# argmaxinc/WhisperKit

Measured on NVIDIA H100. Metric: RTFx (audio-sec/s) whisper-large-v3 greedy, higher is better.
Workload: dtype bf16

## Files before the change

### include/wkb200.h

```cpp
#ifndef WKB200_H
#define WKB200_H

#include <stdint.h>

#ifdef __cplusplus
extern "C" {
#endif

typedef int32_t wk_status;
enum {
    WK_OK = 0,
    WK_ERR_INVALID_ARGUMENT = -1,
    WK_ERR_MODELS_UNAVAILABLE = -2,
    WK_ERR_AUDIO_PROCESSING_FAILED = -3,
    WK_ERR_PREPARE_DECODER_INPUTS = -4,
    WK_ERR_DECODING_LOGITS_FAILED = -5,
    WK_ERR_DECODING_FAILED = -6,
    WK_ERR_TRANSCRIPTION_FAILED = -7,
    WK_ERR_CUDA = -8,
    WK_ERR_LOAD_AUDIO_FAILED = -9
};

typedef struct wk_model wk_model;
typedef struct wk_session wk_session;
// ... 254 lines not shown
                                               int64_t seek, float last_speech_timestamp, float constrained_median, float max_duration,
                                               int32_t special_token_begin, const wk_tokenizer_hooks* hooks, wk_words** out);
wk_status wk_add_word_timestamps(wk_segment* segs, int32_t n_segs, const int32_t* tokens, const float* token_logprobs,
                                 const void* alignment, int32_t dtype, int32_t rows, int32_t cols, int64_t ld,
                                 const wk_tokenizer_hooks* hooks, int64_t seek, float last_speech_timestamp, int32_t special_token_begin,
                                 const char* prepended, const char* appended, wk_words** out);

typedef struct wk_tokenizer wk_tokenizer;
wk_status wk_tokenizer_load(const char* path, wk_tokenizer** out);
wk_status wk_tokenizer_create(const char* const* tokens, const int32_t* ids, const uint8_t* flags, int32_t n, int32_t clean_up_tokenization_spaces,
                              wk_tokenizer** out);
void wk_tokenizer_free(wk_tokenizer* t);
int32_t wk_tokenizer_vocab_size(const wk_tokenizer* t);
int32_t wk_tokenizer_token_to_id(const wk_tokenizer* t, const char* token);
int32_t wk_tokenizer_decode(const wk_tokenizer* t, const int32_t* tokens, int32_t n, int32_t skip_special_tokens, char* text, int32_t cap);
int32_t wk_tokenizer_encode(const wk_tokenizer* t, const char* text_utf8, int32_t* ids, int32_t cap);
wk_status wk_tokenizer_set_merges(wk_tokenizer* t, const char* const* left, const char* const* right, int32_t n);
wk_status wk_tokenizer_special_tokens(const wk_tokenizer* t, wk_special_tokens* out);
int32_t wk_tokenizer_split_to_word_tokens(const wk_tokenizer* t, const int32_t* tokens, int32_t n, char* text, int32_t text_cap, int32_t* counts,
                                          int32_t counts_cap);
wk_status wk_tokenizer_hooks_init(wk_tokenizer* t, wk_tokenizer_hooks* hooks);

int32_t wk_format_time(float seconds, int32_t always_include_hours, const char* decimal_marker, char* out, int32_t cap);
int32_t wk_write_srt(const float* starts, const float* ends, const char* const* texts, int32_t n, char* out, int32_t cap);
int32_t wk_write_vtt(const float* starts, const float* ends, const char* const* texts, int32_t n, char* out, int32_t cap);

int64_t wk_kernel_launch_count(int32_t reset);
wk_status wk_last_timings(wk_model* m, float* ms6);
void* wk_model_stream(wk_model* m);

wk_status wk_test_gemm(wk_model* m, const void* a, const void* w, const float* bias, void* out, int32_t M, int32_t N, int32_t K,
                       int32_t in_dtype, int32_t out_dtype, int32_t gelu);
wk_status wk_test_gemm_residual(wk_model* m, const void* a, const void* w, const float* bias, float* out, int32_t M, int32_t N, int32_t K, int32_t in_dtype);
wk_status wk_test_gemm_splitk(wk_model* m, const void* w, const void* x, float* out, int32_t N, int32_t rows_x, int32_t K, int32_t in_dtype, int32_t splits);
wk_status wk_test_attention(wk_model* m, const void* qkv, void* out, int32_t B, int32_t T, int32_t n_heads, int32_t dtype);
wk_status wk_test_cross_attention(wk_model* m, const float* q, const void* kcross, const void* vcross, void* out, int32_t B, int32_t H,
                                  int32_t T, int32_t dtype, const int32_t* done);
wk_status wk_test_cross_attention_shared(wk_model* m, const float* q, const void* kcross, const void* vcross, void* out, int32_t B, int32_t H,
                                         int32_t T, int32_t dtype, const int32_t* done, int32_t kv_div);
wk_status wk_test_cross_attention_fp8(wk_model* m, const float* q, const uint8_t* kcodes, const uint8_t* vcodes, const float* kscale,
                                      const float* vscale, void* out, int32_t B, int32_t H, int32_t T, int32_t dtype, const int32_t* done,
                                      int32_t kv_div, float* align_out);
wk_status wk_test_self_attention(wk_model* m, const float* qkv, void* kcache, void* vcache, const int32_t* pos, void* out, int32_t B,
                                 int32_t H, int32_t dtype, const int32_t* done);
wk_status wk_test_gemm_partial(wk_model* m, const void* w, const void* x, float* partial_out, int32_t N, int32_t rows_x, int32_t partial_cols,
                               int32_t K, int32_t dtype, int32_t splits);
wk_status wk_test_decoder_reduce(wk_model* m, int32_t kind, const float* partial, int32_t splits, int32_t Bp, const float* bias, const float* gamma,
                                 const float* beta, float* x, void* out16, int32_t B, int32_t n, int32_t dtype);
wk_status wk_test_self_attention_splitk(wk_model* m, const float* partial, int32_t splits, int32_t Bp, const float* bq, const float* bv, void* kcache,
                                        void* vcache, const int32_t* pos, const int32_t* done, const int32_t* anc, void* out, int32_t B, int32_t H,
                                        int32_t dtype);
wk_status wk_test_cross_attention_splitk(wk_model* m, const float* partial, int32_t splits, int32_t Bp, const float* bq, const void* kcross,
                                         const void* vcross, const float* kscale, const float* vscale, void* out, int32_t B, int32_t H, int32_t T,
                                         int32_t dtype, const int32_t* done, int32_t kv_div);

wk_status wk_bench_kernel(wk_model* m, wk_session* s, int32_t which, int32_t batch, int32_t iters, float* ms_out, double* work_out);

wk_status wk_debug_read(wk_model* m, wk_session* s, int32_t which, int64_t offset_elems, float* dst, int64_t n);

#ifdef __cplusplus
}
#endif
#endif
```

### whisperkit_b200/_lib.py

```python
from __future__ import annotations

import ctypes as C
import os

_PKG = os.path.dirname(os.path.abspath(__file__))
LIB_PATH = os.path.join(_PKG, "libwkb200.so")

WK_DTYPE_F32, WK_DTYPE_F16, WK_DTYPE_BF16, WK_DTYPE_I32 = 0, 1, 2, 3
WK_DTYPE_FP8_E4M3 = 4

STATUS_NAMES = {
    0: "ok", -1: "invalidArgument", -2: "modelsUnavailable", -3: "audioProcessingFailed",
    -4: "prepareDecoderInputsFailed", -5: "decodingLogitsFailed", -6: "decodingFailed",
    -7: "transcriptionFailed", -8: "cudaError", -9: "loadAudioFailed",
}
WK_ERR_INVALID_ARGUMENT, WK_ERR_LOAD_AUDIO_FAILED = -1, -9
WK_AUDIO_U8, WK_AUDIO_S16, WK_AUDIO_S24, WK_AUDIO_S32, WK_AUDIO_F32 = 0, 1, 2, 3, 4
WK_CHANNELS_SUM, WK_CHANNELS_SPECIFIC = 0, 1


class WhisperError(RuntimeError):

    def __init__(self, status: int, message: str):
        super().__init__(f"{STATUS_NAMES.get(status, status)}: {message}")
# ... 177 lines not shown
    ("wk_dtw", I32, [P, I32, I32, I32, I64, PI32, PI32, I32, PI32]),
    ("wk_find_alignment", I32, [C.POINTER(wk_word), I32, P, I32, I32, I32, I64, PF32, I32, C.POINTER(P)]),
    ("wk_merge_punctuations", I32, [C.POINTER(wk_word), I32, C.c_char_p, C.c_char_p, C.POINTER(P)]),
    ("wk_word_duration_constraints", I32, [C.POINTER(wk_word), I32, PF32, PF32]),
    ("wk_truncate_long_words", I32, [C.POINTER(wk_word), I32, F32, C.POINTER(P)]),
    ("wk_update_segments_with_word_timings", I32, [C.POINTER(wk_segment), I32, PI32, C.POINTER(wk_word), I32, I64, F32, F32, F32, I32,
                                                   C.POINTER(wk_tokenizer_hooks), C.POINTER(P)]),
    ("wk_add_word_timestamps", I32, [C.POINTER(wk_segment), I32, PI32, PF32, P, I32, I32, I32, I64, C.POINTER(wk_tokenizer_hooks), I64, F32, I32,
                                     C.c_char_p, C.c_char_p, C.POINTER(P)]),
    ("wk_detect_variant", I32, [I32, I32, C.POINTER(C.c_char_p), C.POINTER(C.c_char_p), PI32]),
    ("wk_tokenizer_load", I32, [C.c_char_p, C.POINTER(P)]),
    ("wk_tokenizer_create", I32, [C.POINTER(C.c_char_p), PI32, C.POINTER(C.c_uint8), I32, I32, C.POINTER(P)]),
    ("wk_tokenizer_free", None, [P]),
    ("wk_tokenizer_vocab_size", I32, [P]),
    ("wk_tokenizer_token_to_id", I32, [P, C.c_char_p]),
    ("wk_tokenizer_decode", I32, [P, PI32, I32, I32, C.POINTER(C.c_char), I32]),
    ("wk_tokenizer_encode", I32, [P, C.c_char_p, PI32, I32]),
    ("wk_tokenizer_set_merges", I32, [P, C.POINTER(C.c_char_p), C.POINTER(C.c_char_p), I32]),
    ("wk_tokenizer_special_tokens", I32, [P, C.POINTER(wk_special_tokens)]),
    ("wk_tokenizer_split_to_word_tokens", I32, [P, PI32, I32, C.POINTER(C.c_char), I32, PI32, I32]),
    ("wk_tokenizer_hooks_init", I32, [P, C.POINTER(wk_tokenizer_hooks)]),
    ("wk_format_time", I32, [F32, I32, C.c_char_p, C.POINTER(C.c_char), I32]),
    ("wk_write_srt", I32, [PF32, PF32, C.POINTER(C.c_char_p), I32, C.POINTER(C.c_char), I32]),
    ("wk_write_vtt", I32, [PF32, PF32, C.POINTER(C.c_char_p), I32, C.POINTER(C.c_char), I32]),
    ("wk_kernel_launch_count", I64, [I32]),
    ("wk_last_timings", I32, [P, PF32]),
    ("wk_model_stream", P, [P]),
    ("wk_test_gemm", I32, [P, P, P, P, P, I32, I32, I32, I32, I32, I32]),
    ("wk_test_cross_attention", I32, [P, P, P, P, P, I32, I32, I32, I32, P]),
    ("wk_test_cross_attention_shared", I32, [P, P, P, P, P, I32, I32, I32, I32, P, I32]),
    ("wk_test_cross_attention_fp8", I32, [P, P, P, P, P, P, P, I32, I32, I32, I32, P, I32, P]),
    ("wk_test_self_attention", I32, [P, P, P, P, P, P, I32, I32, I32, P]),
    ("wk_test_gemm_residual", I32, [P, P, P, P, P, I32, I32, I32, I32]),
    ("wk_test_gemm_splitk", I32, [P, P, P, P, I32, I32, I32, I32, I32]),
    ("wk_test_attention", I32, [P, P, P, I32, I32, I32, I32]),
    ("wk_test_gemm_partial", I32, [P, P, P, P, I32, I32, I32, I32, I32, I32]),
    ("wk_test_decoder_reduce", I32, [P, I32, P, I32, I32, P, P, P, P, P, I32, I32, I32]),
    ("wk_test_self_attention_splitk", I32, [P, P, I32, I32, P, P, P, P, P, P, P, P, I32, I32, I32]),
    ("wk_test_cross_attention_splitk", I32, [P, P, I32, I32, P, P, P, P, P, P, I32, I32, I32, I32, P, I32]),
    ("wk_debug_read", I32, [P, P, I32, I64, P, I64]),
    ("wk_bench_kernel", I32, [P, P, I32, I32, I32, PF32, C.POINTER(C.c_double)]),
]

_lib = None


def load() -> C.CDLL:
    global _lib
    if _lib is not None:
        return _lib
    if not os.path.exists(LIB_PATH):
        raise ImportError(
            f"{LIB_PATH} not built: run `python -m whisperkit_b200.build` (needs nvcc). "
            "whisperkit_b200 has no CPU or PyTorch fallback.")
    lib = C.CDLL(LIB_PATH)
    for name, restype, argtypes in SYMBOLS:
        fn = getattr(lib, name)
        fn.restype = restype
        fn.argtypes = argtypes
    _lib = lib
    return lib


def check(status: int) -> None:
    if status != 0:
        raise WhisperError(status, load().wk_last_error().decode("utf-8", "replace"))
# ... 1 lines not shown
```

### whisperkit_b200/csrc/common.cuh

```cuda
#pragma once
#include <cuda.h>
#include <cuda_bf16.h>
#include <cuda_fp16.h>
#include <cuda_fp8.h>
#include <cuda_runtime.h>
#include <stdint.h>
#include <stdio.h>
#include <string.h>

namespace wk {

template <typename T> struct T16;
template <> struct T16<__nv_bfloat16> {
    __device__ __forceinline__ static float to_f(__nv_bfloat16 v) { return __bfloat162float(v); }
    __device__ __forceinline__ static __nv_bfloat16 from_f(float v) { return __float2bfloat16_rn(v); }
    __device__ __forceinline__ static uint32_t pack2(float a, float b) {
        __nv_bfloat162 t = __floats2bfloat162_rn(a, b);
        return *reinterpret_cast<uint32_t*>(&t);
    }
    __device__ __forceinline__ static float2 unpack2(uint32_t u) {
        __nv_bfloat162 t = *reinterpret_cast<__nv_bfloat162*>(&u);
        return __bfloat1622float2(t);
    }
};
// ... 148 lines not shown
}
__device__ __forceinline__ void tma_load_2d_elect(void* smem_dst, const void* tmap, uint64_t* bar, int c0, int c1) {
    asm volatile(
        "{\n\t.reg .pred q;\n\t"
        "elect.sync _|q, 0xffffffff;\n\t"
        "@q cp.async.bulk.tensor.2d.shared::cluster.global.tile.mbarrier::complete_tx::bytes [%0], [%1, {%3, %4}], [%2];\n\t}"
        ::"r"(smem_u32(smem_dst)), "l"(tmap), "r"(smem_u32(bar)), "r"(c0), "r"(c1)
        : "memory");
}
__device__ __forceinline__ void tma_load_3d_elect(void* smem_dst, const void* tmap, uint64_t* bar, int c0, int c1, int c2) {
    asm volatile(
        "{\n\t.reg .pred q;\n\t"
        "elect.sync _|q, 0xffffffff;\n\t"
        "@q cp.async.bulk.tensor.3d.shared::cluster.global.tile.mbarrier::complete_tx::bytes [%0], [%1, {%3, %4, %5}], [%2];\n\t}"
        ::"r"(smem_u32(smem_dst)), "l"(tmap), "r"(smem_u32(bar)), "r"(c0), "r"(c1), "r"(c2)
        : "memory");
}
__device__ __forceinline__ void mbar_expect_tx_elect(uint64_t* bar, uint32_t bytes) {
    asm volatile(
        "{\n\t.reg .pred q;\n\t"
        "elect.sync _|q, 0xffffffff;\n\t"
        "@q mbarrier.arrive.expect_tx.shared::cta.b64 _, [%0], %1;\n\t}" ::"r"(smem_u32(bar)), "r"(bytes)
        : "memory");
}
__device__ __forceinline__ void tma_store_3d(const void* tmap, const void* smem_src, int c0, int c1, int c2) {
    asm volatile("cp.async.bulk.tensor.3d.global.shared::cta.bulk_group [%0, {%2, %3, %4}], [%1];"
                 ::"l"(tmap), "r"(smem_u32(smem_src)), "r"(c0), "r"(c1), "r"(c2)
                 : "memory");
}
__device__ __forceinline__ void bulk_commit() { asm volatile("cp.async.bulk.commit_group;" ::: "memory"); }
__device__ __forceinline__ void bulk_wait_read_all() { asm volatile("cp.async.bulk.wait_group.read 0;" ::: "memory"); }
__device__ __forceinline__ void bulk_wait_all() { asm volatile("cp.async.bulk.wait_group 0;" ::: "memory"); }
__device__ __forceinline__ void warpgroup_bar(int id) { asm volatile("bar.sync %0, 128;" ::"r"(id) : "memory"); }
__device__ __forceinline__ void stmatrix_x4(uint32_t smem_addr, uint32_t r0, uint32_t r1, uint32_t r2, uint32_t r3) {
    asm volatile("stmatrix.sync.aligned.m8n8.x4.shared.b16 [%0], {%1, %2, %3, %4};" ::"r"(smem_addr), "r"(r0), "r"(r1), "r"(r2), "r"(r3)
                 : "memory");
}
__device__ __forceinline__ void bulk_load_1d(void* smem_dst, const void* gsrc, uint32_t bytes, uint64_t* bar) {
    asm volatile(
        "cp.async.bulk.shared::cluster.global.mbarrier::complete_tx::bytes [%0], [%1], %2, [%3];" ::"r"(
            smem_u32(smem_dst)),
        "l"(gsrc), "r"(bytes), "r"(smem_u32(bar))
        : "memory");
}

__device__ __forceinline__ void pdl_launch_dependents() { asm volatile("griddepcontrol.launch_dependents;" ::: "memory"); }
__device__ __forceinline__ void pdl_wait() { asm volatile("griddepcontrol.wait;" ::: "memory"); }

__device__ __forceinline__ void cp_async16(void* smem_dst, const void* gsrc, bool pred) {
    uint32_t sz = pred ? 16u : 0u;
    asm volatile("cp.async.cg.shared.global [%0], [%1], 16, %2;" ::"r"(smem_u32(smem_dst)), "l"(gsrc), "r"(sz)
                 : "memory");
}
__device__ __forceinline__ void cp_async_commit() { asm volatile("cp.async.commit_group;" ::: "memory"); }
template <int N> __device__ __forceinline__ void cp_async_wait() {
    asm volatile("cp.async.wait_group %0;" ::"n"(N) : "memory");
}

bool pdl_enabled();
int pdl_mode();
void pdl_disable();
template <typename... KArgs, typename... Args>
inline cudaError_t launch_k(void (*kernel)(KArgs...), dim3 grid, dim3 block, size_t smem, cudaStream_t stream, int pdl,
                            Args&&... args) {
    cudaLaunchConfig_t cfg;
    memset(&cfg, 0, sizeof(cfg));
// ... 23 lines not shown
```

### whisperkit_b200/csrc/engine.cu

```cuda
#include <math.h>
#include <stdarg.h>
#include <stdio.h>
#include <stdlib.h>
#include <string.h>
#include <dirent.h>

#include <algorithm>
#include <atomic>
#include <map>
#include <string>
#include <vector>

#include "common.cuh"
#include "engine.h"

namespace wk {

static thread_local char g_err[1024] = "";
void set_error(const char* fmt, ...) {
    va_list ap;
    va_start(ap, fmt);
    vsnprintf(g_err, sizeof(g_err), fmt, ap);
    va_end(ap);
}
// ... 884 lines not shown

int64_t wk_kernel_launch_count(int32_t reset) {
    const long long v = wk::launch_counter_load();
    if (reset) wk::launch_counter_sub(v);
    return v;
}

wk_status wk_last_timings(wk_model* m, float* ms6) {
    if (!m || !ms6) return WK_ERR_INVALID_ARGUMENT;
    memcpy(ms6, m->timings, sizeof(m->timings));
    return WK_OK;
}

wk_status wk_test_gemm(wk_model* m, const void* a, const void* w, const float* bias, void* out, int32_t M, int32_t N, int32_t K,
                       int32_t in_dtype, int32_t out_dtype, int32_t gelu) {
    if (!m) return WK_ERR_INVALID_ARGUMENT;
    WK_CUDA_CHECK(cudaSetDevice(m->device));
    std::lock_guard<std::mutex> lock(m->api_mu);
    const int mode = out_dtype == WK_DTYPE_F32 ? GEMM_OUT_F32 : GEMM_OUT_T16;
    WK_CHECK(gemm_wgmma(plain_gemm(a, M, K, w, N, in_dtype, mode, out, N, bias, gelu), m->num_sms, m->stream));
    WK_CUDA_CHECK(cudaStreamSynchronize(m->stream));
    return WK_OK;
}

wk_status wk_test_gemm_residual(wk_model* m, const void* a, const void* w, const float* bias, float* out, int32_t M, int32_t N, int32_t K, int32_t in_dtype) {
    if (!m || !a || !w || !out) return WK_ERR_INVALID_ARGUMENT;
    WK_CUDA_CHECK(cudaSetDevice(m->device));
    std::lock_guard<std::mutex> lock(m->api_mu);
    WK_CHECK(gemm_wgmma(plain_gemm(a, M, K, w, N, in_dtype, GEMM_OUT_F32_ADD, out, N, bias, 0), m->num_sms, m->stream));
    WK_CUDA_CHECK(cudaStreamSynchronize(m->stream));
    return WK_OK;
}

__global__ void reduce_partials_kernel(const float* __restrict__ partial, int splits, int Bp, int N, int rows, float* __restrict__ out) {
    const long long idx = (long long)blockIdx.x * blockDim.x + threadIdx.x;
    if (idx >= (long long)rows * N) return;
    const int b = (int)(idx / N), i = (int)(idx % N);
    float a = 0.f;
    for (int s = 0; s < splits; ++s) a += partial[((long long)s * Bp + b) * N + i];
    out[idx] = a;
}

wk_status wk_test_gemm_splitk(wk_model* m, const void* w, const void* x, float* out, int32_t N, int32_t rows_x, int32_t K, int32_t in_dtype, int32_t splits) {
    if (!m) return WK_ERR_INVALID_ARGUMENT;
    WK_CUDA_CHECK(cudaSetDevice(m->device));
    std::lock_guard<std::mutex> lock(m->api_mu);
    if (rows_x % 16 != 0 || rows_x > 256) { set_error("wk_test_gemm_splitk: rows_x must be a multiple of 16 <= 256"); return WK_ERR_INVALID_ARGUMENT; }
    const int tiles = (N + 127) / 128;
    const int sp = splits > 0 ? splits : choose_splits(tiles, K / 64, m->num_sms);
    float* partial = nullptr;
    WK_CUDA_CHECK(cudaMalloc(&partial, (size_t)sp * rows_x * N * 4));
    GemmDesc g;
    memset(&g, 0, sizeof(g));
    g.a = w; g.a_rows = N; g.a_cols = K; g.a_ld = K; g.a_batches = 1;
    g.b = x; g.b_rows = rows_x; g.b_ld = K; g.in_dtype = in_dtype;
    g.m_rows_per_batch = N; g.n = rows_x; g.k = K; g.taps = 1; g.bn = rows_x; g.splits = sp;
    g.mode = GEMM_OUT_PARTIAL_T; g.out = partial; g.ld_out = N; g.out_rows_per_batch = N; g.partial_cols = rows_x;
    wk_status r = gemm_wgmma(g, m->num_sms, m->stream);
    if (r == WK_OK) {
        const long long n = (long long)rows_x * N;
        reduce_partials_kernel<<<(unsigned)((n + 255) / 256), 256, 0, m->stream>>>(partial, sp, rows_x, N, rows_x, out);
        cudaError_t e = cudaStreamSynchronize(m->stream);
        if (e != cudaSuccess) { set_error("wk_test_gemm_splitk: %s", cudaGetErrorString(e)); r = WK_ERR_CUDA; }
    }
    cudaFree(partial);
    return r;
// ... 145 lines not shown
```

### whisperkit_b200/csrc/gemm_wgmma.cu

```cuda
#include <stdarg.h>
#include <stdio.h>
#include <stdlib.h>

#include <algorithm>

#include "common.cuh"
#include "kernels.h"
#include "wgmma.cuh"

namespace wk {

static constexpr int kBlockM = 128;
static constexpr int kBlockK = 64;
static constexpr int kStageA = kBlockM * kBlockK * 2;
static constexpr int kGemmThreads = 384;
static constexpr int kMaxStages = 10;
static constexpr int kSmemMax = 227 * 1024;

struct GemmKParams {
    int tiles_per_batch, n_batches, tiles_n, splits, work;
    int kb_per_tap, kb_per_split, taps;
    int tap_row_shift[3];
    int tap_col_off[3];
    int a_is_3d;
    int m_rows_per_batch, n, bn;
    int stage_b_bytes, stages, store_bytes;
    int mode, gelu;
    void* out;
    long long ld_out, out_rows_per_batch, partial_cols;
    const float* bias;
    const float* pos;
    long long ld_pos;
    int heads_T, heads_B, heads_H, heads_dmodel;
    float* out_scale;
    int a_static;
};

enum GemmEpi { kEpiPartialT = 0, kEpiFp8Heads = 1, kEpiStore16 = 2, kEpiStore32 = 3 };
static int gemm_epi(int mode) {
    switch (mode) {
        case GEMM_OUT_PARTIAL_T: return kEpiPartialT;
        case GEMM_OUT_FP8_HEADS: return kEpiFp8Heads;
        case GEMM_OUT_T16: case GEMM_OUT_T16_HEADS: return kEpiStore16;
        default: return kEpiStore32;
    }
}

static constexpr int kStoreBox = 64 * 128;
static constexpr int kStoreBytes = 2  * 2  * kStoreBox;

__device__ __forceinline__ uint32_t swz128(int row, int chunk) { return (uint32_t)(row * 128 + ((chunk ^ (row & 7)) << 4)); }

__device__ __forceinline__ void store_box_begin(int wg_tid, int cw) {
    fence_proxy_async();
    if (wg_tid == 0) bulk_wait_read_all();
    warpgroup_bar(1 + cw);
}

template <typename T, int BN>
__device__ __forceinline__ void gemm_epilogue_store16(const GemmKParams& p, const CUtensorMap* tmO, const float (&acc)[BN / 2],
                                                      uint8_t* stage, int& sbuf, int wg_tid, int cw, int batch, int row0, int col_base) {
    const int lane = wg_tid & 31;
    const int q = lane & 3;
    const int mrow = 16 * (wg_tid >> 5) + 8 * ((lane >> 3) & 1) + (lane & 7);
    const int mj = lane >> 4;
    const bool heads = p.mode == GEMM_OUT_T16_HEADS;
    int hb = 0, ht0 = 0;
    bool straddle = false;
// ... 287 lines not shown
            }
            prev = stage;
            if (++stage == p.stages) { stage = 0; phase ^= 1; }
        }
        wgmma_wait<0>();
        __syncwarp();
        if (lane == 0) mbar_arrive(&empty_bar[prev]);

        if constexpr (EPI == kEpiFp8Heads) {
            gemm_epilogue_fp8_heads<BN>(p, batch, tile_row0, r_lo, c_lo, col_base, acc);
        } else if constexpr (EPI == kEpiStore16) {
            if (wg_rows) gemm_epilogue_store16<T, BN>(p, &tmO, acc, my_stage, sbuf, wg_tid, cw, batch, wg_row0, col_base);
        } else if constexpr (EPI == kEpiStore32) {
            if (wg_rows) gemm_epilogue_store32<BN>(p, &tmO, acc, my_stage, my_res_bar, sbuf, rphase, wg_tid, cw, batch, wg_row0, col_base);
        } else {
            float* o = reinterpret_cast<float*>(p.out);
#pragma unroll
            for (int half = 0; half < 2; ++half) {
                const int row_in_batch = tile_row0 + r_lo + 8 * half;
                if (row_in_batch >= p.m_rows_per_batch) continue;
                const long long grow = (long long)batch * p.out_rows_per_batch + row_in_batch;
#pragma unroll
                for (int j = 0; j < BN / 8; ++j) {
                    const int col = col_base + 8 * j + c_lo;
                    if (col < p.partial_cols) o[((long long)split * p.partial_cols + col) * p.ld_out + grow] = acc[4 * j + 2 * half];
                    if (col + 1 < p.partial_cols) o[((long long)split * p.partial_cols + col + 1) * p.ld_out + grow] = acc[4 * j + 2 * half + 1];
                }
            }
        }
    }
    if (kStore && wg_tid == 0) bulk_wait_all();
}

typedef CUresult (*PFN_encodeTiled)(CUtensorMap*, CUtensorMapDataType, cuuint32_t, void*, const cuuint64_t*, const cuuint64_t*,
                                    const cuuint32_t*, const cuuint32_t*, CUtensorMapInterleave, CUtensorMapSwizzle,
                                    CUtensorMapL2promotion, CUtensorMapFloatOOBfill);

static PFN_encodeTiled get_encode_fn() {
    static PFN_encodeTiled fn = nullptr;
    if (!fn) {
        void* p = nullptr;
        cudaDriverEntryPointQueryResult q;
        if (cudaGetDriverEntryPoint("cuTensorMapEncodeTiled", &p, cudaEnableDefault, &q) == cudaSuccess &&
            q == cudaDriverEntryPointSuccess)
            fn = reinterpret_cast<PFN_encodeTiled>(p);
    }
    return fn;
}

static wk_status make_tmap(CUtensorMap* tm, const void* base, int dtype, int ndim, const uint64_t* dims,
                           const uint64_t* strides_bytes, const uint32_t* box) {
    PFN_encodeTiled enc = get_encode_fn();
    if (!enc) {
        set_error("cuTensorMapEncodeTiled entry point unavailable (no CUDA driver?)");
        return WK_ERR_CUDA;
    }
    cuuint64_t gdim[3];
    cuuint64_t gstr[2];
    cuuint32_t bx[3];
    cuuint32_t es[3] = {1, 1, 1};
    for (int i = 0; i < ndim; ++i) { gdim[i] = dims[i]; bx[i] = box[i]; }
    for (int i = 0; i < ndim - 1; ++i) gstr[i] = strides_bytes[i];
    const CUtensorMapDataType ty = dtype == WK_DTYPE_F32 ? CU_TENSOR_MAP_DATA_TYPE_FLOAT32
                                   : dtype == WK_DTYPE_F16 ? CU_TENSOR_MAP_DATA_TYPE_FLOAT16 : CU_TENSOR_MAP_DATA_TYPE_BFLOAT16;
    CUresult r = enc(tm, ty,
                     (cuuint32_t)ndim, const_cast<void*>(base), gdim, gstr, bx, es, CU_TENSOR_MAP_INTERLEAVE_NONE,
// ... 30 lines not shown
        attr_set = true;
    }
    return launch_k(gemm_wgmma_kernel<T, BN, EPI>, dim3(grid), dim3(kGemmThreads), smem, stream, pdl, tmA, tmB, tmO, p);
}

template <typename T, int EPI>
static cudaError_t launch_gemm_store(const CUtensorMap& tmA, const CUtensorMap& tmB, const CUtensorMap& tmO, const GemmKParams& p, int grid,
                                     size_t smem, int pdl, cudaStream_t stream) {
    switch (p.bn) {
        case 64: return launch_gemm<T, 64, EPI>(tmA, tmB, tmO, p, grid, smem, pdl, stream);
        case 128: return launch_gemm<T, 128, EPI>(tmA, tmB, tmO, p, grid, smem, pdl, stream);
        default: return launch_gemm<T, 256, EPI>(tmA, tmB, tmO, p, grid, smem, pdl, stream);
    }
}

template <typename T>
static cudaError_t launch_gemm_n(const CUtensorMap& tmA, const CUtensorMap& tmB, const CUtensorMap& tmO, const GemmKParams& p, int grid,
                                 size_t smem, int pdl, cudaStream_t stream) {
    switch (gemm_epi(p.mode)) {
        case kEpiFp8Heads: return launch_gemm<T, 256, kEpiFp8Heads>(tmA, tmB, tmO, p, grid, smem, pdl, stream);
        case kEpiStore16: return launch_gemm_store<T, kEpiStore16>(tmA, tmB, tmO, p, grid, smem, pdl, stream);
        case kEpiStore32: return launch_gemm_store<T, kEpiStore32>(tmA, tmB, tmO, p, grid, smem, pdl, stream);
        default: break;
    }
    switch (p.bn) {
        case 16: return launch_gemm<T, 16, kEpiPartialT>(tmA, tmB, tmO, p, grid, smem, pdl, stream);
        case 32: return launch_gemm<T, 32, kEpiPartialT>(tmA, tmB, tmO, p, grid, smem, pdl, stream);
        case 64: return launch_gemm<T, 64, kEpiPartialT>(tmA, tmB, tmO, p, grid, smem, pdl, stream);
        case 128: return launch_gemm<T, 128, kEpiPartialT>(tmA, tmB, tmO, p, grid, smem, pdl, stream);
        default: return launch_gemm<T, 256, kEpiPartialT>(tmA, tmB, tmO, p, grid, smem, pdl, stream);
    }
}

wk_status gemm_wgmma(const GemmDesc& d, int num_sms, cudaStream_t stream) {
    if (d.k % kBlockK != 0 || d.bn % 16 != 0 || d.bn < 16 || d.bn > 256 || d.taps < 1 || d.taps > 3) {
        set_error("gemm_wgmma: unsupported shape k=%d bn=%d taps=%d", d.k, d.bn, d.taps);
        return WK_ERR_INVALID_ARGUMENT;
    }
    if (d.mode != GEMM_OUT_PARTIAL_T && (d.n % 32 != 0 || d.splits != 1)) {
        set_error("gemm_wgmma: n=%d must be a multiple of 32 and splits 1 for mode %d", d.n, d.mode);
        return WK_ERR_INVALID_ARGUMENT;
    }
    GemmKParams p;
    memset(&p, 0, sizeof(p));
    p.kb_per_tap = d.k / kBlockK;
    const int total_kb = p.kb_per_tap * d.taps;
    p.splits = d.splits < 1 ? 1 : d.splits;
    if (total_kb % p.splits != 0) {
        set_error("gemm_wgmma: splits %d does not divide %d k-blocks", p.splits, total_kb);
        return WK_ERR_INVALID_ARGUMENT;
    }
    p.kb_per_split = total_kb / p.splits;
    p.taps = d.taps;
    for (int i = 0; i < 3; ++i) { p.tap_row_shift[i] = d.tap_row_shift[i]; p.tap_col_off[i] = d.tap_col_off[i]; }
    p.a_is_3d = d.a_3d ? 1 : 0;
    p.n_batches = d.a_3d ? d.a_batches : 1;
    p.m_rows_per_batch = d.m_rows_per_batch;
    p.tiles_per_batch = (d.m_rows_per_batch + kBlockM - 1) / kBlockM;
    p.n = d.n;
    p.bn = wgmma_tile_n(d.bn);
    const int epi = gemm_epi(d.mode);
    const bool tma_store = epi == kEpiStore16 || epi == kEpiStore32;
    if (tma_store && p.bn < 64) p.bn = 64;
    p.tiles_n = (d.n + p.bn - 1) / p.bn;
    p.work = p.tiles_per_batch * p.n_batches * p.tiles_n * p.splits;
    p.stage_b_bytes = p.bn * kBlockK * 2;
    if (p.stage_b_bytes % 1024 != 0) p.stage_b_bytes = (p.stage_b_bytes + 1023) / 1024 * 1024;
    const int stage_bytes = kStageA + p.stage_b_bytes;
    p.store_bytes = tma_store ? kStoreBytes : 0;
    const int smem_budget = kSmemMax - 1024  - 256  - p.store_bytes;
    int stages = smem_budget / stage_bytes;
    if (stages > kMaxStages) stages = kMaxStages;
    if (stages > total_kb / p.splits + 2) stages = total_kb / p.splits + 2;
    if (stages < 2) stages = 2;
    if (d.max_stages > 0 && stages > d.max_stages) stages = d.max_stages;
    p.stages = stages;
    p.a_static = d.a_static;
    p.mode = d.mode;
    p.gelu = d.gelu;
    p.out = d.out;
    p.ld_out = d.ld_out;
    p.out_rows_per_batch = d.out_rows_per_batch;
    p.partial_cols = d.partial_cols;
    p.bias = d.bias;
    p.pos = d.pos;
    p.ld_pos = d.ld_pos;
    p.heads_T = d.heads_T; p.heads_B = d.heads_B; p.heads_H = d.heads_H; p.heads_dmodel = d.heads_dmodel;
    p.out_scale = d.out_scale;
    if (d.mode == GEMM_OUT_FP8_HEADS && (p.bn != 256 || d.n % 64 != 0 || d.heads_dmodel % 64 != 0 || !d.out_scale)) {
        set_error("gemm_wgmma: the FP8 heads epilogue needs 256-column tiles and head-aligned columns (bn %d n %d d %d)", p.bn, d.n, d.heads_dmodel);
        return WK_ERR_INVALID_ARGUMENT;
    }
    if (d.mode == GEMM_OUT_T16_HEADS &&
        (p.n_batches != 1 || d.n % 64 != 0 || d.heads_dmodel % 64 != 0 || d.n % d.heads_dmodel != 0 || d.m_rows_per_batch % d.heads_T != 0)) {
        set_error("gemm_wgmma: the 16-bit heads epilogue needs head-aligned columns and whole windows (n %d d %d rows %d T %d)", d.n,
                  d.heads_dmodel, d.m_rows_per_batch, d.heads_T);
        return WK_ERR_INVALID_ARGUMENT;
    }

    CUtensorMap tmA, tmB, tmO;
    memset(&tmO, 0, sizeof(tmO));
    wk_status st;
    if (p.a_is_3d) {
        uint64_t dims[3] = {(uint64_t)d.a_cols, (uint64_t)d.a_rows, (uint64_t)d.a_batches};
        uint64_t str[2] = {(uint64_t)d.a_ld * 2, (uint64_t)d.a_batch_stride * 2};
        uint32_t box[3] = {kBlockK, kBlockM, 1};
        st = make_tmap(&tmA, d.a, d.in_dtype, 3, dims, str, box);
    } else {
        uint64_t dims[2] = {(uint64_t)d.a_cols, (uint64_t)d.a_rows};
        uint64_t str[1] = {(uint64_t)d.a_ld * 2};
        uint32_t box[2] = {kBlockK, kBlockM};
        st = make_tmap(&tmA, d.a, d.in_dtype, 2, dims, str, box);
    }
    if (st != WK_OK) return st;
    {
        uint64_t dims[2] = {(uint64_t)d.k * d.taps, (uint64_t)d.b_rows};
        uint64_t str[1] = {(uint64_t)d.b_ld * 2};
        uint32_t box[2] = {kBlockK, (uint32_t)p.bn};
        st = make_tmap(&tmB, d.b, d.in_dtype, 2, dims, str, box);
        if (st != WK_OK) return st;
    }
    if (d.mode == GEMM_OUT_T16_HEADS) {
        uint64_t dims[3] = {64, (uint64_t)d.heads_T, (uint64_t)(d.n / d.heads_dmodel) * d.heads_B * d.heads_H};
        uint64_t str[2] = {128, (uint64_t)d.heads_T * 128};
        uint32_t box[3] = {64, 64, 1};
        st = make_tmap(&tmO, d.out, d.in_dtype, 3, dims, str, box);
    } else if (tma_store) {
        const int out_dtype = epi == kEpiStore16 ? d.in_dtype : WK_DTYPE_F32;
        const uint64_t es = epi == kEpiStore16 ? 2 : 4;
        uint64_t dims[3] = {(uint64_t)d.n, (uint64_t)d.m_rows_per_batch, (uint64_t)p.n_batches};
        uint64_t str[2] = {(uint64_t)d.ld_out * es, (uint64_t)d.out_rows_per_batch * d.ld_out * es};
        uint32_t box[3] = {(uint32_t)(128 / es), 64, 1};
        st = make_tmap(&tmO, d.out, out_dtype, 3, dims, str, box);
    }
    if (st != WK_OK) return st;
    const size_t smem_bytes = (size_t)stages * stage_bytes + p.store_bytes + 1024 + 256;
    int grid = p.work < num_sms ? p.work : num_sms;
    if (grid < 1) return WK_OK;
    const int pdl = d.pdl != 0 ? 16 : 0;
    cudaError_t e = d.in_dtype == WK_DTYPE_F16 ? launch_gemm_n<__half>(tmA, tmB, tmO, p, grid, smem_bytes, pdl, stream)
                                               : launch_gemm_n<__nv_bfloat16>(tmA, tmB, tmO, p, grid, smem_bytes, pdl, stream);
    count_launch();
    if (e == cudaSuccess) e = cudaGetLastError();
    if (e != cudaSuccess) {
        set_error("gemm_wgmma launch: %s", cudaGetErrorString(e));
        return WK_ERR_CUDA;
    }
    return WK_OK;
}

}
```

### whisperkit_b200/csrc/kernels.h

```cpp
#pragma once
#include <cuda.h>
#include <cuda_runtime.h>
#include <stdint.h>

#include "../../include/wkb200.h"

namespace wk {

void set_error(const char* fmt, ...);
const char* last_error_cstr();
void count_launch(int n = 1);

enum GemmMode {
    GEMM_OUT_T16 = 0,
    GEMM_OUT_F32_ADD = 1,
    GEMM_OUT_F32_GELU_POS = 2,
    GEMM_OUT_PARTIAL_T = 3,
    GEMM_OUT_T16_HEADS = 4,
    GEMM_OUT_F32 = 5,
    GEMM_OUT_FP8_HEADS = 6,
};

struct GemmDesc {
    const void* a;
    int64_t a_rows;
    int64_t a_cols;
    int64_t a_ld;
    int64_t a_batch_stride;
    int a_batches;
    int a_3d;
    const void* b;
    int64_t b_rows;
    int64_t b_ld;
    int in_dtype;
    int m_rows_per_batch;
    int n;
    int k;
    int taps;
    int tap_row_shift[3];
    int tap_col_off[3];
    int bn;
    int splits;
    int mode;
    int gelu;
    void* out;
    int64_t ld_out;
    int64_t out_rows_per_batch;
    int64_t partial_cols;
    const float* bias;
    const float* pos;
    int64_t ld_pos;
    int heads_T, heads_B, heads_H, heads_dmodel;
    float* out_scale;
    int pdl;
    int max_stages;
    int a_static;
};

wk_status gemm_wgmma(const GemmDesc& d, int num_sms, cudaStream_t stream);
int wgmma_tile_n(int bn);

struct MelTables;
wk_status mel_tables_create(int n_mels, MelTables** out);
void mel_tables_free(MelTables* t);
wk_status mel_forward(const MelTables* t, const float* pcm, int64_t n_windows, int64_t stride, const int32_t* n_valid,
                      void* out_f16, int32_t* gmax_scratch, cudaStream_t stream);
constexpr int kMelRows = 3002;
constexpr int kMelCols = 128;

wk_status layernorm_f32_to_16(const float* x, const float* gamma, const float* beta, void* out, int64_t rows, int d, int dtype,
                              cudaStream_t stream);
wk_status layernorm_f32_to_f32(const float* x, const float* gamma, const float* beta, float* out, int64_t rows, int d,
                               cudaStream_t stream);
wk_status encoder_attention(const void* qkv, void* out, int B, int T, int n_heads, int dtype, cudaStream_t stream);
wk_status encoder_attention_wgmma(const void* qkv, void* out, int B, int T, int n_heads, int dtype, cudaStream_t stream);
wk_status transpose_to_host_layout(const void* src, float* dst, int64_t B, int64_t rows, int64_t cols, int64_t src_rows_alloc,
                                   int64_t src_row_off, int64_t src_ld, int dtype, cudaStream_t stream);
wk_status fill_random_16(void* dst, int64_t n, uint64_t seed, float std, float mean, int dtype, cudaStream_t stream);
wk_status fill_random_f32(float* dst, int64_t n, uint64_t seed, float std, float mean, cudaStream_t stream);
wk_status convert_to_16(const void* src, int src_dtype, void* dst, int dst_dtype, int64_t n, cudaStream_t stream);

struct RowParams {
    int32_t prompt_len;
    int32_t sample_begin_ts;
    int32_t sample_begin_blank;
    int32_t max_steps;
    float temperature; int32_t top_k;
    int32_t has_first_thr; float first_thr;
    uint64_t seed;
    int32_t suppress_off, n_suppress;
// ... 111 lines not shown
```

Measured before the change: 922.6.

## Add ping-pong warpgroup GEMM schedule for head-output projections

Adds a ping-pong WGMMA GEMM kernel in which two consumer warpgroups take turns on alternate tiles (128x128), coordinated by named barriers. One warpgroup's epilogue then overlaps the other's MMA mainloop, and CTA pairs share B tiles across adjacent M tiles. It is enabled by default for the heads output modes (QKV projections) and can be switched back to cooperative with an environment variable. The cost is a smaller N tile, extra barrier traffic, and more complex scheduling.

```diff
diff --git a/include/wkb200.h b/include/wkb200.h
--- a/include/wkb200.h
+++ b/include/wkb200.h
@@ -310,6 +310,9 @@
 wk_status wk_test_gemm(wk_model* m, const void* a, const void* w, const float* bias, void* out, int32_t M, int32_t N, int32_t K,
                        int32_t in_dtype, int32_t out_dtype, int32_t gelu);
 wk_status wk_test_gemm_residual(wk_model* m, const void* a, const void* w, const float* bias, float* out, int32_t M, int32_t N, int32_t K, int32_t in_dtype);
+wk_status wk_test_gemm_schedule(wk_model* m, int32_t schedule, int32_t mode, const void* a, const void* w, const float* bias, const float* pos,
+                                void* out, float* out_scale, int32_t M, int32_t N, int32_t K, int32_t in_dtype, int32_t gelu, int32_t heads_T,
+                                int32_t heads_B, int32_t heads_H, int32_t heads_dmodel);
 wk_status wk_test_gemm_splitk(wk_model* m, const void* w, const void* x, float* out, int32_t N, int32_t rows_x, int32_t K, int32_t in_dtype, int32_t splits);
 wk_status wk_test_attention(wk_model* m, const void* qkv, void* out, int32_t B, int32_t T, int32_t n_heads, int32_t dtype);
 wk_status wk_test_cross_attention(wk_model* m, const float* q, const void* kcross, const void* vcross, void* out, int32_t B, int32_t H,
diff --git a/whisperkit_b200/_lib.py b/whisperkit_b200/_lib.py
--- a/whisperkit_b200/_lib.py
+++ b/whisperkit_b200/_lib.py
@@ -233,6 +233,7 @@
     ("wk_test_cross_attention_fp8", I32, [P, P, P, P, P, P, P, I32, I32, I32, I32, P, I32, P]),
     ("wk_test_self_attention", I32, [P, P, P, P, P, P, I32, I32, I32, P]),
     ("wk_test_gemm_residual", I32, [P, P, P, P, P, I32, I32, I32, I32]),
+    ("wk_test_gemm_schedule", I32, [P, I32, I32, P, P, P, P, P, P, I32, I32, I32, I32, I32, I32, I32, I32, I32]),
     ("wk_test_gemm_splitk", I32, [P, P, P, P, I32, I32, I32, I32, I32]),
     ("wk_test_attention", I32, [P, P, P, I32, I32, I32, I32]),
     ("wk_test_gemm_partial", I32, [P, P, P, P, I32, I32, I32, I32, I32, I32]),
diff --git a/whisperkit_b200/csrc/common.cuh b/whisperkit_b200/csrc/common.cuh
--- a/whisperkit_b200/csrc/common.cuh
+++ b/whisperkit_b200/csrc/common.cuh
@@ -204,6 +204,8 @@
 __device__ __forceinline__ void bulk_wait_read_all() { asm volatile("cp.async.bulk.wait_group.read 0;" ::: "memory"); }
 __device__ __forceinline__ void bulk_wait_all() { asm volatile("cp.async.bulk.wait_group 0;" ::: "memory"); }
 __device__ __forceinline__ void warpgroup_bar(int id) { asm volatile("bar.sync %0, 128;" ::"r"(id) : "memory"); }
+__device__ __forceinline__ void named_bar_sync(int id, int n) { asm volatile("bar.sync %0, %1;" ::"r"(id), "r"(n) : "memory"); }
+__device__ __forceinline__ void named_bar_arrive(int id, int n) { asm volatile("bar.arrive %0, %1;" ::"r"(id), "r"(n) : "memory"); }
 __device__ __forceinline__ void stmatrix_x4(uint32_t smem_addr, uint32_t r0, uint32_t r1, uint32_t r2, uint32_t r3) {
     asm volatile("stmatrix.sync.aligned.m8n8.x4.shared.b16 [%0], {%1, %2, %3, %4};" ::"r"(smem_addr), "r"(r0), "r"(r1), "r"(r2), "r"(r3)
                  : "memory");
diff --git a/whisperkit_b200/csrc/engine.cu b/whisperkit_b200/csrc/engine.cu
--- a/whisperkit_b200/csrc/engine.cu
+++ b/whisperkit_b200/csrc/engine.cu
@@ -940,6 +940,22 @@
     return WK_OK;
 }
 
+wk_status wk_test_gemm_schedule(wk_model* m, int32_t schedule, int32_t mode, const void* a, const void* w, const float* bias, const float* pos,
+                                void* out, float* out_scale, int32_t M, int32_t N, int32_t K, int32_t in_dtype, int32_t gelu, int32_t heads_T,
+                                int32_t heads_B, int32_t heads_H, int32_t heads_dmodel) {
+    if (!m || !a || !w || !out || mode == GEMM_OUT_PARTIAL_T || mode < 0 || mode > GEMM_OUT_FP8_HEADS) return WK_ERR_INVALID_ARGUMENT;
+    WK_CUDA_CHECK(cudaSetDevice(m->device));
+    std::lock_guard<std::mutex> lock(m->api_mu);
+    GemmDesc g = plain_gemm(a, M, K, w, N, in_dtype, mode, out, N, bias, gelu);
+    g.schedule = schedule;
+    g.pos = pos; g.ld_pos = N;
+    g.heads_T = heads_T; g.heads_B = heads_B; g.heads_H = heads_H; g.heads_dmodel = heads_dmodel;
+    g.out_scale = out_scale;
+    WK_CHECK(gemm_wgmma(g, m->num_sms, m->stream));
+    WK_CUDA_CHECK(cudaStreamSynchronize(m->stream));
+    return WK_OK;
+}
+
 __global__ void reduce_partials_kernel(const float* __restrict__ partial, int splits, int Bp, int N, int rows, float* __restrict__ out) {
     const long long idx = (long long)blockIdx.x * blockDim.x + threadIdx.x;
     if (idx >= (long long)rows * N) return;
diff --git a/whisperkit_b200/csrc/gemm_wgmma.cu b/whisperkit_b200/csrc/gemm_wgmma.cu
--- a/whisperkit_b200/csrc/gemm_wgmma.cu
+++ b/whisperkit_b200/csrc/gemm_wgmma.cu
@@ -34,6 +34,7 @@
     int heads_T, heads_B, heads_H, heads_dmodel;
     float* out_scale;
     int a_static;
+    int b_rows;
 };
 
 enum GemmEpi { kEpiPartialT = 0, kEpiFp8Heads = 1, kEpiStore16 = 2, kEpiStore32 = 3 };
@@ -387,6 +388,151 @@
     if (kStore && wg_tid == 0) bulk_wait_all();
 }
 
+static constexpr int kPpBlockM = 128;
+static constexpr int kPpBN = 128;
+static constexpr int kPpStageA = kPpBlockM * kBlockK * 2;
+static constexpr int kPpStageB = kPpBN * kBlockK * 2;
+static constexpr int kPpTurnBar = 3;
+
+template <typename T, int EPI>
+__global__ void __launch_bounds__(kGemmThreads, 1)
+gemm_wgmma_kernel_pingpong(const __grid_constant__ CUtensorMap tmA, const __grid_constant__ CUtensorMap tmB,
+                           const __grid_constant__ CUtensorMap tmO, const GemmKParams p) {
+    constexpr int BN = kPpBN;
+    constexpr bool kStore = EPI == kEpiStore16 || EPI == kEpiStore32;
+    extern __shared__ __align__(1024) uint8_t smem_raw[];
+    uint8_t* smem = reinterpret_cast<uint8_t*>((reinterpret_cast<uintptr_t>(smem_raw) + 1023) & ~uintptr_t(1023));
+    constexpr int stage_bytes = kPpStageA + kPpStageB;
+    uint8_t* store_stage = smem + (size_t)p.stages * stage_bytes;
+    uint64_t* full_bar = reinterpret_cast<uint64_t*>(store_stage + p.store_bytes);
+    uint64_t* empty_bar = full_bar + kMaxStages;
+    uint64_t* res_bar = empty_bar + kMaxStages;
+
+    const int warp = threadIdx.x >> 5;
+    const int lane = threadIdx.x & 31;
+    const int rank = blockIdx.x & 1;
+    const int pair = blockIdx.x >> 1, n_pairs = gridDim.x >> 1;
+    pdl_launch_dependents();
+
+    if (warp == 0 && lane == 0) {
+        tma_prefetch_desc(&tmA);
+        tma_prefetch_desc(&tmB);
+        if (kStore) tma_prefetch_desc(&tmO);
+        for (int i = 0; i < p.stages; ++i) {
+            mbar_init(&full_bar[i], 1);
+            mbar_init(&empty_bar[i], 4);
+        }
+        for (int i = 0; i < 4; ++i) mbar_init(&res_bar[i], 1);
+        fence_barrier_init();
+    }
+    __syncthreads();
+    pdl_wait();
+
+    if (warp < 4) {
+        asm volatile("setmaxnreg.dec.sync.aligned.u32 40;");
+        if (warp == 0) {
+            int stage = 0;
+            uint32_t phase = 0;
+            for (int w = pair; w < p.work; w += n_pairs) {
+                const int n_tile = w % p.tiles_n;
+                const int m_tile = 2 * (w / p.tiles_n) + rank;
+                const bool valid = m_tile < p.tiles_per_batch;
+                const uint32_t tx = (valid ? kPpStageA : 0) + kPpStageB;
+                for (int kb = 0; kb < p.kb_per_split; ++kb) {
+                    mbar_wait(&empty_bar[stage], phase ^ 1);
+                    __syncwarp();
+                    uint8_t* sa = smem + (size_t)stage * stage_bytes;
+                    mbar_expect_tx_elect(&full_bar[stage], tx);
+                    if (valid) tma_load_2d_elect(sa, &tmA, &full_bar[stage], kb * kBlockK, m_tile * kPpBlockM);
+                    tma_load_2d_elect(sa + kPpStageA, &tmB, &full_bar[stage], kb * kBlockK, n_tile * BN);
+                    if (++stage == p.stages) { stage = 0; phase ^= 1; }
+                }
+            }
+        }
+    } else {
+        asm volatile("setmaxnreg.inc.sync.aligned.u32 232;");
+        const int cw = (warp >> 2) - 1;
+        const int wg_tid = threadIdx.x & 127;
+        const int r_lo = (warp & 3) * 16 + (lane >> 2);
+        const int c_lo = 2 * (lane & 3);
+        uint8_t* my_stage = store_stage + cw * 2 * kStoreBox;
+        uint64_t* my_res_bar = res_bar + 2 * cw;
+        int sbuf = 0;
+        uint32_t rphase = 0;
+        int stage = 0;
+        uint32_t phase = 0;
+        auto release = [&](int st) {
+            __syncwarp();
+            if (lane == 0) mbar_arrive(&empty_bar[st]);
+        };
+        auto prefetch_residual = [&](int r0, int c0) {
+            bulk_wait_read_all();
+            for (int c = 0; c < 2 && c0 + 32 * c < p.n; ++c) {
+                const int b = sbuf ^ c;
+                mbar_expect_tx(&my_res_bar[b], kStoreBox);
+                tma_load_3d(my_stage + b * kStoreBox, &tmO, &my_res_bar[b], c0 + 32 * c, r0, 0);
+            }
+        };
+        float acc[2][BN / 2];
+        int item = 0;
+        for (int w = pair; w < p.work; w += n_pairs, ++item) {
+            if ((item & 1) != cw) {
+                stage += p.kb_per_split;
+                phase ^= (uint32_t)(stage / p.stages) & 1u;
+                stage %= p.stages;
+                continue;
+            }
+            const int n_tile = w % p.tiles_n;
+            const int m_tile = 2 * (w / p.tiles_n) + rank;
+            const bool valid = m_tile < p.tiles_per_batch;
+            const int row0 = m_tile * kPpBlockM;
+            const int col_base = n_tile * BN;
+
+            if (item > 0) named_bar_sync(kPpTurnBar + cw, 256);
+            int prev = -1;
+            for (int kb = 0; kb < p.kb_per_split; ++kb) {
+                mbar_wait(&full_bar[stage], phase);
+                const uint32_t sa = smem_u32(smem + (size_t)stage * stage_bytes);
+                const uint64_t adesc0 = wgmma_desc_sw128(sa), adesc1 = wgmma_desc_sw128(sa + 64 * 128);
+                const uint64_t bdesc = wgmma_desc_sw128(sa + kPpStageA);
+                wgmma_fence();
+#pragma unroll
+                for (int k = 0; k < kBlockK / 16; ++k) {
+                    Wgmma<T, BN>::ss(acc[0], adesc0 + (uint64_t)(2 * k), bdesc + (uint64_t)(2 * k), (kb > 0 || k > 0) ? 1u : 0u);
+                    Wgmma<T, BN>::ss(acc[1], adesc1 + (uint64_t)(2 * k), bdesc + (uint64_t)(2 * k), (kb > 0 || k > 0) ? 1u : 0u);
+                }
+                wgmma_commit();
+                if (EPI == kEpiStore32 && kb == 0 && p.mode == GEMM_OUT_F32_ADD && wg_tid == 0 && valid) {
+                    prefetch_residual(row0, col_base);
+                }
+                wgmma_wait<1>();
+                if (prev >= 0) release(prev);
+                prev = stage;
+                if (++stage == p.stages) { stage = 0; phase ^= 1; }
+            }
+            if (w + n_pairs < p.work) named_bar_arrive(kPpTurnBar + (cw ^ 1), 256);
+            wgmma_wait<0>();
+            release(prev);
+            if (!valid) continue;
+
+#pragma unroll
+            for (int h = 0; h < 2; ++h) {
+                const int hrow0 = row0 + 64 * h;
+                if (hrow0 >= p.m_rows_per_batch) break;
+                if constexpr (EPI == kEpiFp8Heads) {
+                    gemm_epilogue_fp8_heads<BN>(p, 0, hrow0, r_lo, c_lo, col_base, acc[h]);
+                } else if constexpr (EPI == kEpiStore16) {
+                    gemm_epilogue_store16<T, BN>(p, &tmO, acc[h], my_stage, sbuf, wg_tid, cw, 0, hrow0, col_base);
+                } else {
+                    if (h == 1 && p.mode == GEMM_OUT_F32_ADD && wg_tid == 0) prefetch_residual(hrow0, col_base);
+                    gemm_epilogue_store32<BN>(p, &tmO, acc[h], my_stage, my_res_bar, sbuf, rphase, wg_tid, cw, 0, hrow0, col_base);
+                }
+            }
+        }
+        if (kStore && wg_tid == 0) bulk_wait_all();
+    }
+}
+
 typedef CUresult (*PFN_encodeTiled)(CUtensorMap*, CUtensorMapDataType, cuuint32_t, void*, const cuuint64_t*, const cuuint64_t*,
                                     const cuuint32_t*, const cuuint32_t*, CUtensorMapInterleave, CUtensorMapSwizzle,
                                     CUtensorMapL2promotion, CUtensorMapFloatOOBfill);
@@ -483,6 +629,36 @@
     }
 }
 
+template <typename T, int EPI>
+static cudaError_t launch_gemm_pingpong(const CUtensorMap& tmA, const CUtensorMap& tmB, const CUtensorMap& tmO, const GemmKParams& p,
+                                        int grid, size_t smem, int pdl, cudaStream_t stream) {
+    static bool attr_set = false;
+    if (!attr_set) {
+        const cudaError_t e = cudaFuncSetAttribute(gemm_wgmma_kernel_pingpong<T, EPI>, cudaFuncAttributeMaxDynamicSharedMemorySize, kSmemMax);
+        if (e != cudaSuccess) return e;
+        attr_set = true;
+    }
+    return launch_k(gemm_wgmma_kernel_pingpong<T, EPI>, dim3(grid), dim3(kGemmThreads), smem, stream, pdl, tmA, tmB, tmO, p);
+}
+
+template <typename T>
+static cudaError_t launch_gemm_pingpong_n(const CUtensorMap& tmA, const CUtensorMap& tmB, const CUtensorMap& tmO, const GemmKParams& p,
+                                          int grid, size_t smem, int pdl, cudaStream_t stream) {
+    switch (gemm_epi(p.mode)) {
+        case kEpiFp8Heads: return launch_gemm_pingpong<T, kEpiFp8Heads>(tmA, tmB, tmO, p, grid, smem, pdl, stream);
+        case kEpiStore16: return launch_gemm_pingpong<T, kEpiStore16>(tmA, tmB, tmO, p, grid, smem, pdl, stream);
+        default: return launch_gemm_pingpong<T, kEpiStore32>(tmA, tmB, tmO, p, grid, smem, pdl, stream);
+    }
+}
+
+int gemm_schedule_default() {
+    static const int v = [] {
+        const char* e = getenv("WKB200_GEMM_SCHEDULE");
+        return e && strcmp(e, "coop") == 0 ? (int)GEMM_SCHEDULE_COOP : (int)GEMM_SCHEDULE_PINGPONG;
+    }();
+    return v;
+}
+
 wk_status gemm_wgmma(const GemmDesc& d, int num_sms, cudaStream_t stream) {
     if (d.k % kBlockK != 0 || d.bn % 16 != 0 || d.bn < 16 || d.bn > 256 || d.taps < 1 || d.taps > 3) {
         set_error("gemm_wgmma: unsupported shape k=%d bn=%d taps=%d", d.k, d.bn, d.taps);
@@ -507,17 +683,23 @@
     p.a_is_3d = d.a_3d ? 1 : 0;
     p.n_batches = d.a_3d ? d.a_batches : 1;
     p.m_rows_per_batch = d.m_rows_per_batch;
-    p.tiles_per_batch = (d.m_rows_per_batch + kBlockM - 1) / kBlockM;
     p.n = d.n;
     p.bn = wgmma_tile_n(d.bn);
     const int epi = gemm_epi(d.mode);
     const bool tma_store = epi == kEpiStore16 || epi == kEpiStore32;
     if (tma_store && p.bn < 64) p.bn = 64;
+    const bool heads = d.mode == GEMM_OUT_T16_HEADS || d.mode == GEMM_OUT_FP8_HEADS;
+    const int sched = d.schedule ? d.schedule : heads ? gemm_schedule_default() : (int)GEMM_SCHEDULE_COOP;
+    const bool pp = sched == GEMM_SCHEDULE_PINGPONG && epi != kEpiPartialT && !p.a_is_3d && d.taps == 1 && p.bn == 256;
+    const int coop_bn = p.bn;
+    if (pp) p.bn = kPpBN;
+    const int block_m = pp ? kPpBlockM : kBlockM;
+    p.tiles_per_batch = (d.m_rows_per_batch + block_m - 1) / block_m;
     p.tiles_n = (d.n + p.bn - 1) / p.bn;
-    p.work = p.tiles_per_batch * p.n_batches * p.tiles_n * p.splits;
+    p.work = pp ? (p.tiles_per_batch + 1) / 2 * p.tiles_n : p.tiles_per_batch * p.n_batches * p.tiles_n * p.splits;
     p.stage_b_bytes = p.bn * kBlockK * 2;
     if (p.stage_b_bytes % 1024 != 0) p.stage_b_bytes = (p.stage_b_bytes + 1023) / 1024 * 1024;
-    const int stage_bytes = kStageA + p.stage_b_bytes;
+    const int stage_bytes = (pp ? kPpStageA : kStageA) + p.stage_b_bytes;
     p.store_bytes = tma_store ? kStoreBytes : 0;
     const int smem_budget = kSmemMax - 1024  - 256  - p.store_bytes;
     int stages = smem_budget / stage_bytes;
@@ -527,6 +709,7 @@
     if (d.max_stages > 0 && stages > d.max_stages) stages = d.max_stages;
     p.stages = stages;
     p.a_static = d.a_static;
+    p.b_rows = (int)d.b_rows;
     p.mode = d.mode;
     p.gelu = d.gelu;
     p.out = d.out;
@@ -538,7 +721,7 @@
     p.ld_pos = d.ld_pos;
     p.heads_T = d.heads_T; p.heads_B = d.heads_B; p.heads_H = d.heads_H; p.heads_dmodel = d.heads_dmodel;
     p.out_scale = d.out_scale;
-    if (d.mode == GEMM_OUT_FP8_HEADS && (p.bn != 256 || d.n % 64 != 0 || d.heads_dmodel % 64 != 0 || !d.out_scale)) {
+    if (d.mode == GEMM_OUT_FP8_HEADS && (coop_bn != 256 || d.n % 64 != 0 || d.heads_dmodel % 64 != 0 || !d.out_scale)) {
         set_error("gemm_wgmma: the FP8 heads epilogue needs 256-column tiles and head-aligned columns (bn %d n %d d %d)", p.bn, d.n, d.heads_dmodel);
         return WK_ERR_INVALID_ARGUMENT;
     }
@@ -560,7 +743,7 @@
     } else {
         uint64_t dims[2] = {(uint64_t)d.a_cols, (uint64_t)d.a_rows};
         uint64_t str[1] = {(uint64_t)d.a_ld * 2};
-        uint32_t box[2] = {kBlockK, kBlockM};
+        uint32_t box[2] = {kBlockK, (uint32_t)block_m};
         st = make_tmap(&tmA, d.a, d.in_dtype, 2, dims, str, box);
     }
     if (st != WK_OK) return st;
@@ -586,11 +769,18 @@
     }
     if (st != WK_OK) return st;
     const size_t smem_bytes = (size_t)stages * stage_bytes + p.store_bytes + 1024 + 256;
-    int grid = p.work < num_sms ? p.work : num_sms;
-    if (grid < 1) return WK_OK;
+    if (p.work < 1) return WK_OK;
     const int pdl = d.pdl != 0 ? 16 : 0;
-    cudaError_t e = d.in_dtype == WK_DTYPE_F16 ? launch_gemm_n<__half>(tmA, tmB, tmO, p, grid, smem_bytes, pdl, stream)
-                                               : launch_gemm_n<__nv_bfloat16>(tmA, tmB, tmO, p, grid, smem_bytes, pdl, stream);
+    cudaError_t e;
+    if (pp) {
+        const int grid = 2 * (p.work < num_sms / 2 ? p.work : num_sms / 2);
+        e = d.in_dtype == WK_DTYPE_F16 ? launch_gemm_pingpong_n<__half>(tmA, tmB, tmO, p, grid, smem_bytes, pdl, stream)
+                                       : launch_gemm_pingpong_n<__nv_bfloat16>(tmA, tmB, tmO, p, grid, smem_bytes, pdl, stream);
+    } else {
+        const int grid = p.work < num_sms ? p.work : num_sms;
+        e = d.in_dtype == WK_DTYPE_F16 ? launch_gemm_n<__half>(tmA, tmB, tmO, p, grid, smem_bytes, pdl, stream)
+                                       : launch_gemm_n<__nv_bfloat16>(tmA, tmB, tmO, p, grid, smem_bytes, pdl, stream);
+    }
     count_launch();
     if (e == cudaSuccess) e = cudaGetLastError();
     if (e != cudaSuccess) {
diff --git a/whisperkit_b200/csrc/kernels.h b/whisperkit_b200/csrc/kernels.h
--- a/whisperkit_b200/csrc/kernels.h
+++ b/whisperkit_b200/csrc/kernels.h
@@ -55,7 +55,10 @@
     int pdl;
     int max_stages;
     int a_static;
-};
+    int schedule;
+};
+enum GemmSchedule { GEMM_SCHEDULE_COOP = 1, GEMM_SCHEDULE_PINGPONG = 2 };
+int gemm_schedule_default();
 
 wk_status gemm_wgmma(const GemmDesc& d, int num_sms, cudaStream_t stream);
 int wgmma_tile_n(int bn);
```

After: 924.0 (median of 6 runs). About the same (+0.2%).
